# tuanir/fantoch

Hardware: AMD Instinct MI355X
Metric: region configs evaluated/sec (1/2/4/8 GPUs), synthetic 64-region planet n=7 f=1,2 (higher is better)
Workload: dtype u32

## Files before the change

fantoch_amd/csrc/bote_capi.hip:

```cpp
#include <hip/hip_runtime.h>

#include <algorithm>
#include <cmath>
#include <cstring>
#include <mutex>
#include <string>
#include <map>
#include <memory>
#include <vector>

#include "../../include/bote_hip.h"
#include "bote_host.hpp"
#include "bote_kernels.hpp"

using bote::EvalArgs;
using bote::Rec;
using bote::SingleArgs;

using namespace bote::host;

namespace {

thread_local std::string g_err;

// ... 85 lines not shown
  const bote_planet* p = nullptr;
  uint32_t n = 0, ns = 0, nc = 0, n_obj = 0, K = 0;
  EvalArgs args{};
  uint32_t grid = 0, bd = 0;
  size_t shm = 0;
  DBuf srv, cli, binom, top, tmp0, tmp1, result, counters;
  DBuf top_alt, counters_alt;
  hipEvent_t ev0 = nullptr, ev1 = nullptr;
  hipEvent_t last0 = nullptr, last1 = nullptr;
  hipEvent_t done = nullptr;
  std::vector<std::pair<hipEvent_t, hipEvent_t>> evpool;
  size_t ev_used = 0;
  bool launched = false;
  bool fast = false;
  bool group = false;
  bool def_obj = false;
  bote::FastArgs fargs{};
  uint32_t fgrid = 0;
  size_t fshm = 0;
  uint32_t xgrid = 0;
  DBuf cqt, rqt, queue, qcount, lowtab;
  DBuf dbg;
  DBuf pstats;
  struct Chunks {
    std::vector<uint64_t> host;
    std::vector<uint64_t> state;
    DBuf dev, sdev;
    uint32_t n = 0;
  };
  std::map<std::pair<uint64_t, uint64_t>, std::unique_ptr<Chunks>> chunks;
  std::map<std::pair<uint64_t, uint64_t>, std::unique_ptr<Chunks>> samples;
  DBuf smin, tseed;
  DBuf kbound;
  mutable std::vector<std::shared_ptr<const GroupWalk>> walks;
  DBuf wctr;
  uint64_t last_rb = 0, last_re = 0;
  hipStream_t last_stream = nullptr;
  uint64_t result_bytes() const { return (uint64_t)n_obj * bote::KP * 16 + 16; }
};

namespace {
constexpr uint64_t QUEUE_CAP = 1ull << 20;

#ifndef BOTE_CHUNKS_PER_WAVE
#define BOTE_CHUNKS_PER_WAVE 32
#endif
}

struct DevGuard {
  int dev = -1;
  DevGuard() {
    if (hipGetDevice(&dev) != hipSuccess) dev = -1;
  }
  ~DevGuard() {
    if (dev >= 0) (void)hipSetDevice(dev);
  }
  DevGuard(const DevGuard&) = delete;
  DevGuard& operator=(const DevGuard&) = delete;
};

extern "C" {

const char* bote_last_error(void) { return g_err.c_str(); }

int bote_device_count(int* out) {
  if (!out) return fail(BOTE_E_ARG, "out is null");
// ... 894 lines not shown
  s->last0 = e0 ? *e0 : s->ev0;
  s->last1 = e1 ? *e1 : s->ev1;
  HIP_TRY(hipEventRecord(s->last0, st));
  HIP_TRY(bote::launch_eval(a, s->n, false, s->grid, s->bd, s->shm, st));
  HIP_TRY(hipEventRecord(s->last1, st));
  return merge_chain(s, s->grid, st);
}

static int sample_seed(bote_sweep* s, bote::FastArgs& f, uint64_t rb, uint64_t re, hipStream_t st) {
  const uint32_t nwaves = s->fgrid * (s->fargs.gbd / 64);
  const uint32_t nsamp = sample_count(rb, re, binom_u64(s->ns, s->n), nwaves, s->K);
  if (!nsamp) return BOTE_OK;
  auto key = std::make_pair(rb, re);
  auto it = s->samples.find(key);
  if (it == s->samples.end()) {
    if (s->samples.size() >= 16) {
      if (s->last_stream) HIP_TRY(hipStreamSynchronize(s->last_stream));
      HIP_TRY(hipStreamSynchronize(st));
      s->samples.clear();
    }
    if (s->n - 3 > 16) return BOTE_OK;
    auto c = std::make_unique<bote_sweep::Chunks>();
    c->n = nsamp;
    c->host = sample_starts(rb, re, nsamp);
    if (!chunk_states(c->host.data(), nsamp, s->n, s->ns, c->state)) return fail(BOTE_E_ARG, "sample rank out of range");
    if (c->dev.alloc(c->host.size() * 8) != hipSuccess || c->sdev.alloc(c->state.size() * 8) != hipSuccess)
      return fail(BOTE_E_NOMEM, "hipMalloc sample chunks");
    HIP_TRY(hipMemcpyAsync(c->dev.p, c->host.data(), c->host.size() * 8, hipMemcpyHostToDevice, st));
    HIP_TRY(hipMemcpyAsync(c->sdev.p, c->state.data(), c->state.size() * 8, hipMemcpyHostToDevice, st));
    it = s->samples.emplace(key, std::move(c)).first;
  }
  const bote_sweep::Chunks* c = it->second.get();
  const uint32_t slots = nwaves >= s->K ? nwaves : nsamp;
  if (s->smin.reserve((size_t)s->n_obj * slots * 8) != hipSuccess || s->tseed.reserve(bote::MAXOBJ * 8) != hipSuccess)
    return fail(BOTE_E_NOMEM, "hipMalloc top-K seed");
  if (slots != nwaves || slots == nsamp) HIP_TRY(hipMemsetAsync(s->smin.p, 0xFF, (size_t)s->n_obj * slots * 8, st));
  bote::FastArgs fs = f;
  fs.smin = s->smin.as<uint64_t>();
  fs.tseed = nullptr;
  fs.wchunks = c->dev.as<uint64_t>();
  fs.wstate = c->sdev.as<uint64_t>();
  fs.nwchunks = nsamp;
  fs.ssteps = 1;
  fs.smin_wave = slots == nwaves && slots != nsamp ? 1u : 0u;
  fs.wctr = f.wctr + 256;
  HIP_TRY(bote::launch_group(fs, s->n, s->def_obj, s->fgrid, s->fshm, st));
  HIP_TRY(bote::launch_seed(fs.smin, fs.smin_wave ? nwaves : nsamp, s->n_obj, s->K, s->tseed.as<uint64_t>(), st));
  f.tseed = s->tseed.as<uint64_t>();
  return BOTE_OK;
}

static int launch_fast_path(bote_sweep* s, uint64_t rb, uint64_t re, hipStream_t st) {
  bote::FastArgs f = s->fargs;
  f.rb = rb;
  f.re = re;
  f.runlen = sweep_runlen(re - rb, s->fgrid, bote::FAST_BD);
  if (s->group) {
    const bote_sweep::Chunks* ch = nullptr;
    int crc = sweep_chunks(s, rb, re, st, &ch);
    if (crc) return crc;
    f.nwchunks = ch ? ch->n : 0;
    f.wchunks = ch ? ch->dev.as<uint64_t>() : nullptr;
    f.wstate = ch && !ch->state.empty() ? ch->sdev.as<uint64_t>() : nullptr;
    if (f.nwchunks) {
      if (!s->wctr.p && s->wctr.alloc(16 * 128) != hipSuccess) return fail(BOTE_E_NOMEM, "hipMalloc work counters");
      f.wctr = s->wctr.as<unsigned int>();
      f.wshards = s->fgrid % 8 == 0 ? 8u : 1u;
    }
  }
  f.kbound = nullptr;
  if (s->group && s->n_obj && s->K && wide_merge(s->fgrid + s->xgrid, s->grid)) {
    if (!s->kbound.p && s->kbound.alloc(bote::MAXOBJ * 8) != hipSuccess) return fail(BOTE_E_NOMEM, "hipMalloc K-th key bound");
    f.kbound = s->kbound.as<unsigned long long>();
  }
  HIP_TRY(bote::launch_zero_ctl(s->counters.as<unsigned long long>(), s->qcount.as<unsigned long long>(),
                                f.nwchunks ? f.wctr : nullptr, s->counters_alt.as<unsigned long long>(), f.kbound, st));
  if (s->group && f.nwchunks && s->n_obj && s->K) {
    int src = sample_seed(s, f, rb, re, st);
    if (src) return src;
  }
  hipEvent_t *e0 = nullptr, *e1 = nullptr;
  int rc;
  if ((rc = timing_slot(s, e0, e1))) return rc;
  s->last0 = *e0;
  s->last1 = *e1;
  if (s->group) HIP_TRY(bote::launch_group(f, s->n, s->def_obj, s->fgrid, s->fshm, st, *e0, *e1));
  else HIP_TRY(bote::launch_fast(f, s->n, s->fgrid, s->fshm, st, *e0, *e1));
  EvalArgs a = s->args;
  a.rank_list = s->queue.as<uint64_t>();
  a.rank_count = s->qcount.as<unsigned long long>();
  a.rb = 0;
  a.re = QUEUE_CAP;
  a.runlen = 1;
  a.out_top = s->n_obj ? s->top.as<Rec>() + (size_t)s->fgrid * s->n_obj * bote::KP : nullptr;
  HIP_TRY(bote::launch_eval(a, s->n, false, s->xgrid, s->bd, s->shm, st));
  EvalArgs g = s->args;
  g.rb = rb;
  g.re = re;
  g.runlen = sweep_runlen(re - rb, s->grid, s->bd);
  g.out_top = s->n_obj ? s->top_alt.as<Rec>() : nullptr;
  g.out_counters = s->counters_alt.as<unsigned long long>();
  g.run_if_over = s->qcount.as<unsigned long long>();
  g.over_cap = QUEUE_CAP;
  HIP_TRY(bote::launch_eval(g, s->n, false, s->grid, s->bd, s->shm, st));
  return merge_chain(s, s->fgrid + s->xgrid, st, s->qcount.as<unsigned long long>(), s->grid, f.kbound);
}

int bote_sweep_launch(bote_sweep* s, uint64_t rank_begin, uint64_t rank_end, void* hip_stream) {
  DevGuard dev_guard;
// ... 382 lines not shown
```

fantoch_amd/csrc/bote_group.hip:

```cpp
#include "bote_fast.hpp"
#include "bote_launch.hpp"

#define AS3 __attribute__((address_space(3)))

namespace bote {

constexpr int GROUP_MAX_BD = 1024;
#ifndef BOTE_GROUP_WAVES
#define BOTE_GROUP_WAVES 5
#endif
#ifndef BOTE_GROUP_WAVES_PERM
#define BOTE_GROUP_WAVES_PERM 4
#endif

__host__ __device__ constexpr int cmax(int a, int b) { return a > b ? a : b; }
template <bool B>
struct BoolC {
  static constexpr bool value = B;
};

template <int N>
struct GCfg {
  using QC = QCfg<N>;
  static constexpr int F = N - 3;
// ... 174 lines not shown
  return (float)__longlong_as_double((long long)tkey) * (1.0f + 0x1p-10f);
}

template <int KA, int KY, class T>
__device__ __forceinline__ void merge_top4(const T* A, const T* y, T* L) {
  static_assert(KA >= 1 && KY >= 1 && KA + KY >= 4 && KA <= 4 && KY <= 4, "4 smallest of KA + KY >= 4 entries");
  T B[4];
#pragma unroll
  for (int i = 0; i < 4; ++i) {
    const int j = 3 - i;
    if (i < KA && j < KY) B[i] = __builtin_elementwise_min(A[i < KA ? i : 0], y[j < KY ? j : 0]);
    else if (i < KA) B[i] = A[i < KA ? i : 0];
    else B[i] = y[j < KY ? j : 0];
  }
  auto ce = [&](int a, int b) {
    const T lo = __builtin_elementwise_min(B[a], B[b]);
    B[b] = __builtin_elementwise_max(B[a], B[b]);
    B[a] = lo;
  };
  ce(0, 2);
  ce(1, 3);
  ce(0, 1);
  ce(2, 3);
#pragma unroll
  for (int i = 0; i < 4; ++i) L[i] = B[i];
}

template <int KA, int KY, int KO, class T>
__device__ __forceinline__ void merge_k(const T* A, const T* y, T* L) {
  if constexpr (KO == 4 && KA + KY >= 4) merge_top4<KA, KY>(A, y, L);
  else merge_lists<KA, KY, KO>(A, y, L);
}

__device__ __forceinline__ void wave_topk(const TopkLds& t, int* lock, uint32_t nc, int n_obj, uint32_t K,
                                          const uint64_t (&key)[MAXOBJ], const bool (&ok)[MAXOBJ], uint64_t rank) {
  const uint32_t lane = threadIdx.x & 63;
  const int KL = (int)K;
  if (lane == 0) {
    while (atomicCAS(lock, 0, 1) != 0) __builtin_amdgcn_s_sleep(2);
  }
  __builtin_amdgcn_wave_barrier();
  __builtin_amdgcn_fence(__ATOMIC_ACQUIRE, "workgroup");
  const uint32_t rlo = (uint32_t)rank, rhi = (uint32_t)(rank >> 32);
#pragma unroll
  for (int o = 0; o < MAXOBJ; ++o) {
    if (o >= n_obj) break;
    Rec* top = t.top + o * KL;
    const Rec mine = Rec{key[o], rank};
    const bool p = ok[o] && rec_lt(mine, t.thr[o]);
    const uint64_t m = __ballot(p);
    if (m == 0) continue;
    const bool h0 = (int)lane < KL, h1 = (int)lane + 64 < KL;
    const Rec x0 = h0 ? top[lane] : rec_max(), x1 = h1 ? top[lane + 64] : rec_max();
    int r0 = (int)lane, r1 = (int)lane + 64;
    int rc = p ? lower_bound_rec(top, KL, mine) : 0;
    const uint32_t klo = (uint32_t)key[o], khi = (uint32_t)(key[o] >> 32);
    for (uint64_t mm = m; mm; mm &= mm - 1) {
      const int src = __builtin_ctzll(mm);
      const uint64_t ck = ((uint64_t)(uint32_t)__builtin_amdgcn_readlane(khi, src) << 32) |
                          (uint32_t)__builtin_amdgcn_readlane(klo, src);
      const uint64_t cr = ((uint64_t)(uint32_t)__builtin_amdgcn_readlane(rhi, src) << 32) |
                          (uint32_t)__builtin_amdgcn_readlane(rlo, src);
      const Rec c = Rec{ck, cr};
      r0 += rec_lt(c, x0);
      r1 += rec_lt(c, x1);
      rc += rec_lt(c, mine);
    }
    if (h0 && r0 < KL) t.tmp[r0] = x0;
    if (h1 && r1 < KL) t.tmp[r1] = x1;
    if (p && rc < KL) t.tmp[rc] = mine;
    wave_sync();
#pragma unroll
    for (int h = 0; h < KP / 64; ++h)
      if ((int)lane + 64 * h < KL) top[lane + 64 * h] = t.tmp[lane + 64 * h];
    wave_sync();
    if (lane == 0 && rec_lt(top[K - 1], t.thr[o])) {
      t.thr[o] = top[K - 1];
      if (o == 0) lock[1] = score_tlo(top[K - 1].key, nc);
      if (o == 3) lock[2] = __float_as_int(cov_tf32(top[K - 1].key));
    }
    wave_sync();
  }
  __builtin_amdgcn_fence(__ATOMIC_RELEASE, "workgroup");
  if (lane == 0) atomicExch(lock, 0);
}

template <class FX, class FY>
__device__ __forceinline__ int cov2_sign(float Vx, uint32_t Sx, float Vy, uint32_t Sy, const FX& dVx, const FY& dVy) {
  const float fx = (float)Sx, fy = (float)Sy;
  const float x = Vx * (fy * fy), y = Vy * (fx * fx);
  const float d = x - y, tol = 0x1p-18f * fmaxf(x, y);
  if (d < -tol) return -1;
  if (d > tol) return 1;
  const double sx = (double)Sx, sy = (double)Sy;
  const double X = dVx() * (sy * sy), Y = dVy() * (sx * sx);
  const double D = X - Y, T = 0x1p-32 * fmax(X, Y);
  return D < -T ? -1 : (D > T ? 1 : 0);
}

template <class FX, class FY>
__device__ __forceinline__ int cov2_sign_ge(float Vx, uint32_t Sx, float Vy, uint32_t Sy, const FX& dVx, const FY& dVy) {
  const float fx = (float)Sx, fy = (float)Sy;
  const float x = Vx * (fy * fy), y = Vy * (fx * fx);
  constexpr float c = 1.0f - 0x1p-18f;
  if (x * c >= y) return 1;
  if (x < y * c) return -1;
  const double sx = (double)Sx, sy = (double)Sy;
  const double X = dVx() * (sy * sy), Y = dVy() * (sx * sx);
  const double D = X - Y, T = 0x1p-32 * fmax(X, Y);
  return D < -T ? -1 : (D > T ? 1 : 0);
}

__device__ __forceinline__ float u64_to_f32(uint64_t x) {
  return __builtin_fmaf((float)(uint32_t)(x >> 32), 0x1p32f, (float)(uint32_t)x);
}

constexpr uint32_t GROUP_UNROLL = 4;
#ifndef BOTE_BIN_FIRST
#define BOTE_BIN_FIRST 0
#endif
#ifndef BOTE_BIN_FIRST_XK
#define BOTE_BIN_FIRST_XK 1
#endif
constexpr uint32_t BIN_UB = 4;
template <int N, bool DEF, bool SI, bool RXC, bool XK, bool BN = false>
__global__ void __launch_bounds__(XK ? GROUP_XK_MAX_BD : GROUP_MAX_BD,
                                  XK ? BOTE_GROUP_WAVES_XK : (GCfg<N>::PERM ? BOTE_GROUP_WAVES_PERM : BOTE_GROUP_WAVES))
    sweep_group_kernel(FastArgs a) {
  const bool sid = SI || a.srv_identity;
  constexpr bool S32 = SI;
  const bool use_rx = GCfg<N>::RX && (SI ? RXC : a.grx != 0);
  using QC = QCfg<N>;
  using GC = GCfg<N>;
  constexpr int NL = QC::NL;
  constexpr int NLW = NL <= 2 ? 1 : 2;
  constexpr int F = GC::F;
  constexpr int FP = GC::FP;
  constexpr int KQ = GC::KQ;
  constexpr int PV = Pow2<N - 1>::v;
  constexpr int PF = Pow2<F>::v;
  constexpr bool PERM = GC::PERM;
  constexpr bool BIN = XK || (PERM && BN);
  constexpr bool BIN_FIRST = BIN && (XK ? BOTE_BIN_FIRST_XK : BOTE_BIN_FIRST);
  static_assert(!XK || (PERM && DEF), "the extended key set runs on the PERM kernels with the default objectives");
  using QT = QTab<N, XK>;
  constexpr int NT = QT::NT;
  extern __shared__ __align__(16) unsigned char smem[];
  size_t off[16];
  group_layout(a, N, NLW, KQ, PERM, off);
  const uint32_t LB = lds_base(smem);
  const uint32_t qtab = LB + (uint32_t)off[0];
  const uint32_t cqt = LB + (uint32_t)off[1];
  const uint32_t rqt = LB + (uint32_t)(a.rq_separate ? off[2] : off[1]);
  uint32_t* srv = (uint32_t*)(smem + off[3]);
  uint2* lrec = (uint2*)(smem + off[4]);
  uint64_t* cs2 = (uint64_t*)(smem + off[5]);
  double* vcol = (double*)(smem + off[6]);
  float* vcol32 = (float*)(smem + off[7]);
  const uint64_t* binom = a.binom;
  TopkLds tk;
  tk.top = (Rec*)(smem + off[9]);
  tk.cand = (Rec*)(smem + off[10]);
  tk.tmp = (Rec*)(smem + off[11]);
// ... 50 lines not shown
  __syncthreads();

  const uint32_t nc = a.nc, nq = nc >> 2, rem = nc & 3;
  const uint32_t qlane = qtab + tid * 4;
  const uint32_t lines = qtab + wid * lines_wave_bytes(a);
  const uint32_t keys = lines + a.gslots * cstride;
  const uint32_t gl = LB + (uint32_t)off[8] + wid * gline_bytes(a, N, KQ);
  const uint32_t rxt = gl;
  const uint32_t mfl = gl + gline_rx_bytes(a, N);
  const uint32_t upk = mfl + cstride;
  const uint32_t fS1 = upk + FP * KQ * 4;
  const uint32_t fVf = fS1 + F * 4;
  const double pnc1 = a.p_fmean * (double)nc, pnc2 = a.p_emean * (double)nc;
  uint64_t valid_cnt = 0;
  const uint32_t dofs = uni(LB + (uint32_t)off[15] + wid * 512u - 2u * (LB + (uint32_t)off[14] + wid * (N * 256u)));
  auto digest_add = [&](uint32_t binb_, uint64_t d) {
    uint32_t ad;
    asm("v_lshl_add_u32 %0, %1, 1, %2" : "=v"(ad) : "v"(binb_), "s"(dofs));
    __hip_atomic_fetch_add((AS3 uint64_t*)(uintptr_t)ad, d, __ATOMIC_RELAXED, __HIP_MEMORY_SCOPE_WAVEFRONT);
  };

  bool static_done = false;
  const uint32_t wsh = a.wshards ? a.wshards : 1u, wx = blockIdx.x % wsh;
  unsigned int* const tctr = a.wctr + 32 * wx;
  uint32_t cnext = 0;
  if (a.nwchunks && lane == 0) cnext = atomicAdd(tctr, 1u);
  for (;;) {
  uint64_t r, rend;
  uint32_t chunk = ~0u;
  if (a.nwchunks) {
    const uint32_t c = wx + wsh * uni(cnext);
    if (c >= a.nwchunks) break;
    if (lane == 0) cnext = atomicAdd(tctr, 1u);
    chunk = c;
    PSTAT(a, 13, true);
    r = uni64(a.wchunks[c]);
    rend = a.smin ? min(r + 64ull * a.ssteps, a.re) : uni64(a.wchunks[c + 1]);
    GASSERT(a, a.rb <= r && r <= rend && rend <= a.re, 0);
  } else {
    if (static_done) break;
    static_done = true;
    const uint64_t nwaves = (uint64_t)gridDim.x * WPB;
    const uint64_t gw = (uint64_t)blockIdx.x * WPB + wid;
    const uint64_t total = a.re - a.rb;
    r = uni64(a.rb + (uint64_t)(((unsigned __int128)total * gw) / nwaves));
    rend = uni64(a.rb + (uint64_t)(((unsigned __int128)total * (gw + 1)) / nwaves));
  }

  if (r < rend) {
    uint32_t hq[F];
    uint64_t base = 0;
    if (a.wstate && chunk != ~0u) {
      const uint64_t* st = a.wstate + 4 * (size_t)chunk;
      base = uni64(st[0]);
      const uint64_t b0 = uni64(st[1]), b1 = uni64(st[2]);
#pragma unroll
      for (int k = 0; k < F; ++k) hq[k] = (uint32_t)((k < 8 ? b0 >> (8 * k) : b1 >> (8 * (k - 8))) & 0xFFu);
    } else {
      uint32_t p[N];
      colex_unrank<N>(binom, a.ns, r, p);
#pragma unroll
      for (int k = 0; k < F; ++k) {
        hq[k] = uni(p[3 + k]);
        base += binom[hq[k] * (N + 1) + (k + 4)];
      }
      base = uni64(base);
// ... 1053 lines not shown
        if (a.smin) {
          const int nobj = XK ? 8 : (DEF ? 5 : a.n_obj);
#pragma unroll
          for (int o = 0; o < MAXOBJ; ++o) {
            if (o >= nobj) break;
            uint64_t v = ok[o] ? key[o] : ~0ull;
#pragma unroll
            for (int d = 32; d >= 1; d >>= 1) {
              const uint64_t w = ((uint64_t)(uint32_t)__shfl_xor((int)(v >> 32), d) << 32) |
                                 (uint32_t)__shfl_xor((int)(uint32_t)v, d);
              v = w < v ? w : v;
            }
            uint32_t ch = uni(chunk);
            asm volatile("" : "+s"(ch));
            const size_t slot = a.smin_wave ? (size_t)o * gridDim.x * WPB + (size_t)blockIdx.x * WPB + wid
                                            : (size_t)o * a.nwchunks + ch;
            if (lane == (a.smin_wave ? (uint32_t)o : 0u) && v != ~0ull)
              atomicMin((unsigned long long*)&a.smin[slot], v);
          }
        } else if (!ABLATE(a, 4)) {
          const int nobj = XK ? 8 : (DEF ? 5 : a.n_obj);
          uint64_t th[MAXOBJ];
#pragma unroll
          for (int o = 0; o < MAXOBJ; ++o)
            if (o < nobj) {
              const uint2 t = l64(thra + 16u * o);
              th[o] = ((uint64_t)t.y << 32) | t.x;
            }
          bool pass = false;
#pragma unroll
          for (int o = 0; o < MAXOBJ; ++o)
            if (o < nobj) pass = pass || (ok[o] && key[o] <= th[o]);
          PSTAT(a, 11, pass);
          if (__ballot(pass)) wave_topk(tk, lock, a.nc, nobj, a.K, key, ok, rank);
        }
        r += len;
        left -= len;
      }
      if (r >= rend || a.smin) break;
      {
        int js = F;
#pragma unroll
        for (int k = F - 1; k >= 0; --k) {
          const uint32_t nxt = (k == F - 1) ? a.ns : hq[k + 1];
          if (hq[k] + 1 < nxt) js = k;
        }
        base = 0;
#pragma unroll
        for (int k = 0; k < F; ++k) {
          hq[k] = uni(k < js ? (uint32_t)(3 + k) : (k == js ? hq[k] + 1 : hq[k]));
          base += binom[hq[k] * (N + 1) + (k + 4)];
        }
        base = uni64(base);
        low = 0;
      }
      wave_sync();
    }
  }
  wave_sync();
  }
  if (a.smin) return;
  if (valid_cnt && lane == 0) atomicAdd(&a.out_counters[0], (unsigned long long)valid_cnt);
  const uint64_t digest = *(const AS3 uint64_t*)(uintptr_t)(LB + (uint32_t)off[15] + tid * 8);
  if (digest) atomicAdd(&a.out_counters[1], (unsigned long long)digest);
  __syncthreads();
  Rec* dst = a.out_top + (size_t)blockIdx.x * a.n_obj * KP;
  if (a.kbound) {
    if (tid < a.n_obj) {
      const Rec kth = tk.top[tid * a.K + a.K - 1];
      uint64_t b = ~0ull;
      if (!(kth.key == ~0ull && kth.rank == ~0ull)) {
        b = atomicMin(&a.kbound[tid], (unsigned long long)kth.key);
        b = b < kth.key ? b : kth.key;
      } else {
        b = __hip_atomic_load(&a.kbound[tid], __ATOMIC_RELAXED, __HIP_MEMORY_SCOPE_AGENT);
      }
      tk.thr[tid].key = b;
    }
    __syncthreads();
    for (uint32_t i = tid; i < (uint32_t)a.n_obj * a.K; i += BD) {
      const uint32_t o = i / a.K, e = i % a.K;
      const uint64_t b = tk.thr[o].key;
      const Rec r = tk.top[i];
      const bool in = !(r.key == ~0ull && r.rank == ~0ull) && r.key <= b;
      bool prev = true;
      if (e) {
        const Rec q = tk.top[i - 1];
        prev = !(q.key == ~0ull && q.rank == ~0ull) && q.key <= b;
      }
      if (in) dst[o * KP + e] = r;
      else if (prev) dst[o * KP + e] = rec_max();
    }
    return;
  }
  for (uint32_t i = tid; i < (uint32_t)a.n_obj * KP; i += BD) {
    const uint32_t o = i / KP, e = i % KP;
    dst[i] = e < a.K ? tk.top[o * a.K + e] : rec_max();
  }
}

static bool group_si(const FastArgs& a) { return a.srv_identity && a.want_digest && a.ft_metric == 2 && a.s32 && a.v32; }

bool group_supports_keys(uint32_t n, uint32_t bd) { return n >= 4 && n <= 7 && group_uses_lines(n) && bd <= GROUP_XK_MAX_BD; }

template <int N, bool XK>
static const void* group_fn_n(const FastArgs& a, bool def) {
  if constexpr (XK) {
    return group_si(a) ? (a.grx ? (const void*)sweep_group_kernel<N, true, true, true, true>
                                : (const void*)sweep_group_kernel<N, true, true, false, true>)
// ... 45 lines not shown
```

fantoch_amd/csrc/bote_kernels.hip:

```cpp
#include <atomic>
#include "bote_kernels.hpp"
#include "bote_launch.hpp"

namespace bote {

struct Smem {
  uint32_t* mat;
  uint32_t* clioff;
  uint32_t* srv;
  uint64_t* cs;
  uint64_t* binom;
  uint32_t* qtab;
  TopkLds tk;
};

__host__ __device__ inline size_t align_up(size_t x, size_t a) { return (x + a - 1) / a * a; }

__host__ __device__ inline size_t smem_layout(const EvalArgs& a, int N, int NLW, uint32_t BD, bool topk,
                                              size_t* off) {
  size_t o = 0;
  off[0] = o; o += (size_t)a.R * a.R * 4;
  off[1] = o; o += (size_t)a.nc * 4;
  off[2] = o; o += (size_t)a.ns * 4;
  o = align_up(o, 16);
// ... 1016 lines not shown
  __syncthreads();
  for (uint32_t i = tid; i < (uint32_t)KP; i += WIDE_BD) out[i] = i < have && i < KK ? buf[i] : rec_max();
}
#undef WIDE_T

hipError_t launch_merge_wide(const Rec* src, uint32_t n_lists, const Rec* alt, uint32_t alt_lists, uint64_t list_stride,
                             const unsigned long long* sel, uint64_t cap, const unsigned long long* kbound, Rec* dst,
                             uint32_t n_obj, uint32_t K, const unsigned long long* csrc, const unsigned long long* calt,
                             uint64_t* cdst, hipStream_t st) {
  if (n_lists > (uint32_t)(WIDE_BD * WIDE_LISTS_PER_THREAD) || alt_lists > (uint32_t)(WIDE_BD * WIDE_LISTS_PER_THREAD))
    return hipErrorInvalidValue;
  const size_t shm = merge_wide_smem();
  static std::atomic<uint64_t> done{0};
  int dev = 0;
  hipError_t e = hipGetDevice(&dev);
  if (e != hipSuccess) return e;
  const uint64_t bit = 1ull << (dev & 63);
  if (!(done.load(std::memory_order_relaxed) & bit)) {
    e = hipFuncSetAttribute((const void*)merge_wide_kernel, hipFuncAttributeMaxDynamicSharedMemorySize, (int)shm);
    if (e != hipSuccess) return e;
    done.fetch_or(bit, std::memory_order_relaxed);
  }
  hipLaunchKernelGGL(merge_wide_kernel, dim3(n_obj), dim3(WIDE_BD), shm, st, src, n_lists, list_stride, dst, alt,
                     alt_lists, sel, cap, kbound, K, csrc, calt, cdst);
  return hipGetLastError();
}

__global__ void pick_counters_kernel(const unsigned long long* src, const unsigned long long* alt,
                                     const unsigned long long* sel, uint64_t cap, uint64_t* dst) {
  if (threadIdx.x < 2) dst[threadIdx.x] = (*sel > cap ? alt : src)[threadIdx.x];
}

__global__ void zero_ctl_kernel(unsigned long long* counters, unsigned long long* qcount, unsigned int* wctr,
                                unsigned long long* counters_alt, unsigned long long* kbound) {
  const uint32_t t = threadIdx.x;
  if (t < 2) counters[t] = 0;
  if (t == 2) *qcount = 0;
  if (t >= 4 && t < 6) counters_alt[t - 4] = 0;
  if (t >= 8 && t < 24 && wctr) wctr[32 * (t - 8)] = 0;
  if (t >= 32 && t < 32 + MAXOBJ && kbound) kbound[t - 32] = ~0ull;
}

hipError_t launch_zero_ctl(unsigned long long* counters, unsigned long long* qcount, unsigned int* wctr,
                           unsigned long long* counters_alt, unsigned long long* kbound, hipStream_t st) {
  hipLaunchKernelGGL(zero_ctl_kernel, dim3(1), dim3(64), 0, st, counters, qcount, wctr, counters_alt, kbound);
  return hipGetLastError();
}

__global__ void __launch_bounds__(1024) seed_kernel(const uint64_t* smin, uint32_t nsamp, uint32_t K, uint64_t* tseed) {
  __shared__ uint32_t hist[256];
  __shared__ uint64_t sel[3];
  __shared__ uint64_t red[2][16];
  __shared__ uint64_t few[64];
  __shared__ uint32_t nfew;
  const uint32_t o = blockIdx.x, tid = threadIdx.x, BD = blockDim.x;
  if (nsamp < K || K == 0) {
    if (tid == 0) tseed[o] = ~0ull;
    return;
  }
  const uint64_t* x = smin + (size_t)o * nsamp;
  constexpr int RP = 32;
  const bool inreg = nsamp <= (uint32_t)RP * BD;
  uint64_t xr[RP];
#pragma unroll
  for (int i = 0; i < RP; ++i) {
    const uint32_t k = tid + (uint32_t)i * BD;
    xr[i] = inreg && k < nsamp ? x[k] : ~0ull;
  }
  uint64_t va = ~0ull, vo = 0;
  if (inreg) {
#pragma unroll
    for (int i = 0; i < RP; ++i)
      if (tid + (uint32_t)i * BD < nsamp) {
        va &= xr[i];
        vo |= xr[i];
      }
  } else {
    for (uint32_t k = tid; k < nsamp; k += BD) {
      va &= x[k];
      vo |= x[k];
    }
  }
#pragma unroll
  for (int d = 32; d >= 1; d >>= 1) {
    va &= (uint64_t)__shfl_xor((long long)va, d);
    vo |= (uint64_t)__shfl_xor((long long)vo, d);
  }
  if ((tid & 63) == 0) {
    red[0][tid >> 6] = va;
    red[1][tid >> 6] = vo;
  }
  __syncthreads();
  if (tid == 0) {
    uint64_t a = ~0ull, b = 0;
    for (uint32_t w = 0; w < (BD >> 6); ++w) {
      a &= red[0][w];
      b |= red[1][w];
    }
    const uint64_t diff = a ^ b;
    const int top = diff ? 63 - __clzll(diff) : -1;
    const int pass0 = top < 0 ? -1 : top / 8;
    sel[0] = pass0 < 0 ? a : (pass0 == 7 ? 0 : a >> (8 * (pass0 + 1)));
    sel[1] = K;
    red[0][0] = (uint64_t)(int64_t)pass0;
  }
  __syncthreads();
  const int pass0 = (int)(int64_t)red[0][0];
  for (int pass = pass0; pass >= 0; --pass) {
    if (tid < 256) hist[tid] = 0;
    __syncthreads();
    const uint64_t prefix = sel[0];
    const int sh = 8 * pass;
    auto count = [&](uint64_t v) {
      if (pass == 7 || (v >> (sh + 8)) == prefix) atomicAdd(&hist[(v >> sh) & 0xFFu], 1u);
    };
    if (inreg) {
#pragma unroll
      for (int i = 0; i < RP; ++i)
        if (tid + (uint32_t)i * BD < nsamp) count(xr[i]);
    } else {
      for (uint32_t k = tid; k < nsamp; k += BD) count(x[k]);
    }
    __syncthreads();
    if (tid < 64) {
      uint32_t c[4], s = 0;
#pragma unroll
      for (int b = 0; b < 4; ++b) c[b] = hist[4 * tid + b];
#pragma unroll
      for (int b = 0; b < 4; ++b) s += c[b];
      uint32_t incl = s;
#pragma unroll
      for (int d = 1; d < 64; d <<= 1) {
        const uint32_t y = __shfl_up(incl, d);
        if ((int)tid >= d) incl += y;
      }
      const uint64_t need = sel[1];
      uint32_t before = incl - s;
      int digit = -1;
      uint64_t left = 0;
#pragma unroll
// ... 8 lines not shown
        sel[0] = (sel[0] << 8) | (uint64_t)digit;
        sel[1] = left;
        sel[2] = hist[digit];
      }
      if (tid == 0) nfew = 0;
    }
    __syncthreads();
    if (pass > 0 && sel[2] <= 64) {
      const uint64_t pfx = sel[0];
      const int shb = 8 * pass;
      auto push = [&](uint64_t v) {
        if ((v >> shb) == pfx) few[atomicAdd(&nfew, 1u)] = v;
      };
      if (inreg) {
#pragma unroll
        for (int i = 0; i < RP; ++i)
          if (tid + (uint32_t)i * BD < nsamp) push(xr[i]);
      } else {
        for (uint32_t k = tid; k < nsamp; k += BD) push(x[k]);
      }
      __syncthreads();
      if (tid < 64) {
        const uint32_t nb = nfew, need = (uint32_t)sel[1];
        const uint64_t v = tid < nb ? few[tid] : ~0ull;
        uint32_t lt = 0, le = 0;
        for (uint32_t j = 0; j < nb; j += 4) {
#pragma unroll
          for (uint32_t u = 0; u < 4; ++u) {
            const uint64_t y = few[j + u];
            lt += (uint32_t)(j + u < nb && y < v);
            le += (uint32_t)(j + u < nb && y <= v);
          }
        }
        if (tid < nb && lt < need && need <= le) tseed[o] = v;
      }
      return;
    }
  }
  if (tid == 0) tseed[o] = sel[0];
}

hipError_t launch_seed(const uint64_t* smin, uint32_t nsamp, uint32_t n_obj, uint32_t K, uint64_t* tseed,
                       hipStream_t st) {
  hipLaunchKernelGGL(seed_kernel, dim3(n_obj), dim3(1024), 0, st, smin, nsamp, K, tseed);
  return hipGetLastError();
}

hipError_t launch_pick_counters(const unsigned long long* src, const unsigned long long* alt,
                                const unsigned long long* sel, uint64_t cap, uint64_t* dst, hipStream_t st) {
  hipLaunchKernelGGL(pick_counters_kernel, dim3(1), dim3(64), 0, st, src, alt, sel, cap, dst);
  return hipGetLastError();
}

__global__ void sum_counters_kernel(const uint64_t* src, uint32_t n, uint64_t stride, uint64_t off, uint64_t* dst) {
  if (threadIdx.x < 2) {
    uint64_t s = 0;
    for (uint32_t i = 0; i < n; ++i) s += src[i * stride + off + threadIdx.x];
    dst[threadIdx.x] = s;
  }
}

hipError_t launch_sum_counters(const uint64_t* src, uint32_t n, uint64_t stride, uint64_t off, uint64_t* dst,
                               hipStream_t st) {
  hipLaunchKernelGGL(sum_counters_kernel, dim3(1), dim3(64), 0, st, src, n, stride, off, dst);
  return hipGetLastError();
}

hipError_t launch_single(const SingleArgs& a, int mode, hipStream_t st) {
  size_t shm = align_up((size_t)a.R * a.R * 4 + a.R, 16) + (size_t)a.R * 4;
  hipError_t e = hipFuncSetAttribute((const void*)single_kernel, hipFuncAttributeMaxDynamicSharedMemorySize, (int)shm);
  if (e != hipSuccess) return e;
  hipLaunchKernelGGL(single_kernel, dim3(1), dim3(256), shm, st, a, mode);
// ... 10 lines not shown
```

fantoch_amd/csrc/bote_kernels.hpp:

```cpp
#pragma once
#include "bote_device.hpp"

namespace bote {

constexpr int NSLOT = 10;
constexpr int G_MERGE_LISTS = 8;
enum { SLOT_AF1 = 0, SLOT_FF1 = 1, SLOT_AF2 = 2, SLOT_FF2 = 3, SLOT_E = 4 };
enum { OBJ_SCORE = 0, OBJ_MEAN = 1, OBJ_COV = 2 };

struct EvalArgs {
  const uint32_t* mat;
  uint32_t R;
  const uint32_t* srv;
  uint32_t ns;
  const uint32_t* cli;
  uint32_t nc;
  int srv_sorted;
  const uint32_t* cfgs;
  const uint64_t* rank_list;
  const unsigned long long* rank_count;
  uint64_t rb, re;
  uint32_t runlen;
  const uint64_t* binom;
  int want_score;
  double p_fmean, p_emean, p_fair;
  int ft_metric;
  uint32_t keys;
  uint32_t* out_vals;
  uint32_t* out_leader;
  uint64_t* out_s1;
  uint64_t* out_s2;
  double* out_mean;
  double* out_cov;
// ... 34 lines not shown
  const uint2* cqt;
  const uint2* rqt;
  int rq_separate;
  uint32_t R, cq_quads, rq_quads;
  uint32_t cq_stride, rq_stride;
  const uint32_t* srv;
  uint32_t ns;
  int srv_identity;
  uint32_t nc;
  const uint64_t* binom;
  uint64_t rb, re;
  uint32_t runlen;
  uint32_t s2_flush;
  uint32_t g_flush;
  uint32_t k_flush;
  uint32_t gbd;
  uint32_t gqsh;
  uint32_t gslots;
  uint32_t grx;
  uint32_t keys;
  uint32_t gbins;
  uint32_t s32;
  uint32_t v32;
  const uint64_t* wchunks;
  uint32_t nwchunks;
  unsigned int* wctr;
  uint32_t wshards;
  const uint64_t* wstate;
  uint64_t* smin;
  const uint64_t* tseed;
  uint32_t ssteps;
  uint32_t smin_wave;
  unsigned long long* kbound;
  int want_score, p_int;
  int64_t p1i, p2i;
  int32_t m1_lo, m1_hi, m2_lo, m2_hi;
  double p_fmean, p_emean;
  int ft_metric;
  int n_obj;
  uint32_t obj_kind[MAXOBJ];
  uint32_t obj_slot[MAXOBJ];
  uint32_t K;
  Rec* out_top;
  unsigned long long* out_counters;
  int want_digest;
  const uint32_t* lowtab;
  uint64_t* queue;
  unsigned long long* queue_count;
  uint64_t queue_cap;
#ifdef BOTE_DEBUG
  unsigned int* dbg_flag;
  uint64_t lowtab_n;
#endif
#ifdef BOTE_PATHSTATS
  unsigned long long* pstats;
#endif
#ifdef BOTE_ABLATION
  uint32_t ablate;
#endif
};
#ifdef BOTE_DEBUG
#define GASSERT(a, cond, code)                                                    \
  do {                                                                            \
    if (!(cond)) atomicOr((a).dbg_flag, 1u << (code));                            \
  } while (0)
#else
// ... 17 lines not shown
#else
#define ABLATE(a, bit) false
#endif
size_t fast_smem_bytes(const FastArgs& a, uint32_t n);
int fast_occupancy(uint32_t n, size_t shm);
hipError_t launch_fast(const FastArgs& a, uint32_t n, uint32_t grid, size_t shm, hipStream_t st, hipEvent_t e0 = nullptr,
                       hipEvent_t e1 = nullptr);
size_t group_smem_bytes(const FastArgs& a, uint32_t n);
bool group_uses_lines(uint32_t n);
#ifndef BOTE_GROUP_WAVES_XK
#define BOTE_GROUP_WAVES_XK 4
#endif
constexpr uint32_t GROUP_XK_MAX_BD = 256 * BOTE_GROUP_WAVES_XK;
bool group_supports_keys(uint32_t n, uint32_t bd);
int group_occupancy(const FastArgs& a, uint32_t n, size_t shm, bool def_objectives);
hipError_t launch_group(const FastArgs& a, uint32_t n, bool def_objectives, uint32_t grid, size_t shm, hipStream_t st,
                        hipEvent_t e0 = nullptr, hipEvent_t e1 = nullptr);

size_t eval_smem_bytes(const EvalArgs& a, uint32_t n, uint32_t bd, bool topk);
int eval_occupancy(uint32_t n, bool full, uint32_t bd, size_t shm, bool keys = false);
hipError_t launch_eval(const EvalArgs& a, uint32_t n, bool full, uint32_t grid, uint32_t bd, size_t shm,
                       hipStream_t st);
hipError_t launch_merge(const Rec* src, uint32_t n_lists, uint64_t list_stride, Rec* dst, uint64_t out_stride,
                        uint32_t n_obj, hipStream_t st);
constexpr uint32_t WIDE_MERGE_LISTS = 4096;
hipError_t launch_merge_wide(const Rec* src, uint32_t n_lists, const Rec* alt, uint32_t alt_lists, uint64_t list_stride,
                             const unsigned long long* sel, uint64_t cap, const unsigned long long* kbound, Rec* dst,
                             uint32_t n_obj, uint32_t K, const unsigned long long* csrc, const unsigned long long* calt,
                             uint64_t* cdst, hipStream_t st);
hipError_t launch_merge_sel(const Rec* src, uint32_t n_lists, const Rec* alt, uint32_t alt_lists, uint64_t list_stride,
                            const unsigned long long* sel, uint64_t cap, Rec* dst, uint64_t out_stride, uint32_t n_obj,
                            hipStream_t st);
hipError_t launch_zero_ctl(unsigned long long* counters, unsigned long long* qcount, unsigned int* wctr,
                           unsigned long long* counters_alt, unsigned long long* kbound, hipStream_t st);
hipError_t launch_seed(const uint64_t* smin, uint32_t nsamp, uint32_t n_obj, uint32_t K, uint64_t* tseed,
                       hipStream_t st);
hipError_t launch_pick_counters(const unsigned long long* src, const unsigned long long* alt,
                                const unsigned long long* sel, uint64_t cap, uint64_t* dst, hipStream_t st);

hipError_t launch_sum_counters(const uint64_t* src, uint32_t n, uint64_t stride, uint64_t off, uint64_t* dst,
                               hipStream_t st);
struct LqArgs {
  const uint32_t* mat;
  uint32_t R;
  const uint32_t* srv;
  uint32_t ns;
  const uint32_t* cli;
  uint32_t nc;
  const uint32_t* cfgs;
  const uint64_t* binom;
  uint64_t rank_begin, ncfg;
  const uint32_t* qs;
  uint32_t nq;
  uint32_t* out_vals;
  uint64_t* out_sum;
  uint64_t* out_sumsq;
};
size_t lq_smem_bytes(const LqArgs& a, uint32_t n);
hipError_t launch_leaderless_q(const LqArgs& a, uint32_t n, uint32_t grid, size_t shm, hipStream_t st);

struct ChainHostLevel {
  uint32_t cnt, n;
  const uint64_t* mask;
  const double* score;
  const double* mean;
};
hipError_t chain_search(const ChainHostLevel* lv, uint32_t ns, int ft_metric, double min_dec, uint64_t max_out,
// ... 7 lines not shown
```

Measured before the change: 48.83 billion.

## Share a device-wide key histogram to tighten per-workgroup top-K thresholds

```diff
diff --git a/fantoch_amd/csrc/bote_bound.hpp b/fantoch_amd/csrc/bote_bound.hpp
--- /dev/null
+++ b/fantoch_amd/csrc/bote_bound.hpp
@@ -0,0 +1,56 @@
+#pragma once
+#include <cstdint>
+
+#if defined(__HIPCC__) || defined(__CUDACC__)
+#define BOTE_HD __host__ __device__ inline
+#else
+#define BOTE_HD inline
+#endif
+
+namespace bote {
+
+constexpr uint32_t BOUND_NB = 256;
+constexpr uint32_t BOUND_OFF = 64;
+
+struct BoundPlan {
+  uint64_t base;
+  uint64_t top;
+  uint32_t shift;
+};
+
+BOTE_HD BoundPlan bound_plan(uint64_t base, uint64_t top) {
+  BoundPlan p{base, top, BOUND_OFF};
+  if (top == ~0ull || base > top) return p;
+  const uint64_t d = top - base;
+  uint32_t s = 0;
+  while (s < 63 && (d >> s) > BOUND_NB - 1) ++s;
+  p.shift = s;
+  return p;
+}
+
+BOTE_HD bool bound_on(const BoundPlan& p) { return p.shift < BOUND_OFF; }
+
+BOTE_HD uint32_t bound_bin(const BoundPlan& p, uint64_t k) {
+  if (!bound_on(p) || k <= p.base) return 0;
+  const uint64_t j = (k - p.base) >> p.shift;
+  return j < BOUND_NB - 1 ? (uint32_t)j : BOUND_NB - 1;
+}
+
+BOTE_HD uint64_t bound_edge(const BoundPlan& p, uint32_t j) {
+  if (!bound_on(p)) return ~0ull;
+  const uint64_t jt = (p.top - p.base) >> p.shift;
+  if (j >= jt) return p.top;
+  return p.base + (((uint64_t)j + 1) << p.shift) - 1;
+}
+
+BOTE_HD uint64_t bound_from_hist(const BoundPlan& p, const uint32_t* hist, uint32_t K) {
+  if (!bound_on(p) || K == 0) return ~0ull;
+  uint64_t sum = 0;
+  for (uint32_t j = 0; j < BOUND_NB; ++j) {
+    sum += hist[j];
+    if (sum >= K) return bound_edge(p, j);
+  }
+  return ~0ull;
+}
+
+}
diff --git a/fantoch_amd/csrc/bote_capi.hip b/fantoch_amd/csrc/bote_capi.hip
--- a/fantoch_amd/csrc/bote_capi.hip
+++ b/fantoch_amd/csrc/bote_capi.hip
@@ -141,6 +141,7 @@
   std::map<std::pair<uint64_t, uint64_t>, std::unique_ptr<Chunks>> samples;
   DBuf smin, tseed;
   DBuf kbound;
+  DBuf bhist;
   mutable std::vector<std::shared_ptr<const GroupWalk>> walks;
   DBuf wctr;
   uint64_t last_rb = 0, last_re = 0;
@@ -1101,7 +1102,7 @@
   }
   const bote_sweep::Chunks* c = it->second.get();
   const uint32_t slots = nwaves >= s->K ? nwaves : nsamp;
-  if (s->smin.reserve((size_t)s->n_obj * slots * 8) != hipSuccess || s->tseed.reserve(bote::MAXOBJ * 8) != hipSuccess)
+  if (s->smin.reserve((size_t)s->n_obj * slots * 8) != hipSuccess || s->tseed.reserve(3 * bote::MAXOBJ * 8) != hipSuccess)
     return fail(BOTE_E_NOMEM, "hipMalloc top-K seed");
   if (slots != nwaves || slots == nsamp) HIP_TRY(hipMemsetAsync(s->smin.p, 0xFF, (size_t)s->n_obj * slots * 8, st));
   bote::FastArgs fs = f;
@@ -1142,8 +1143,15 @@
     if (!s->kbound.p && s->kbound.alloc(bote::MAXOBJ * 8) != hipSuccess) return fail(BOTE_E_NOMEM, "hipMalloc K-th key bound");
     f.kbound = s->kbound.as<unsigned long long>();
   }
+  f.bhist = nullptr;
+  if (s->group && f.nwchunks && s->n_obj && s->K) {
+    if (!s->bhist.p && s->bhist.alloc(bote::MAXOBJ * bote::BOUND_NB * 4) != hipSuccess)
+      return fail(BOTE_E_NOMEM, "hipMalloc key bound histograms");
+    f.bhist = s->bhist.as<unsigned int>();
+  }
   HIP_TRY(bote::launch_zero_ctl(s->counters.as<unsigned long long>(), s->qcount.as<unsigned long long>(),
-                                f.nwchunks ? f.wctr : nullptr, s->counters_alt.as<unsigned long long>(), f.kbound, st));
+                                f.nwchunks ? f.wctr : nullptr, s->counters_alt.as<unsigned long long>(), f.kbound, f.bhist,
+                                st));
   if (s->group && f.nwchunks && s->n_obj && s->K) {
     int src = sample_seed(s, f, rb, re, st);
     if (src) return src;
diff --git a/fantoch_amd/csrc/bote_group.hip b/fantoch_amd/csrc/bote_group.hip
--- a/fantoch_amd/csrc/bote_group.hip
+++ b/fantoch_amd/csrc/bote_group.hip
@@ -230,10 +230,93 @@
   else merge_lists<KA, KY, KO>(A, y, L);
 }
 
+__device__ __forceinline__ BoundPlan load_plan(const uint64_t* plan, int o) {
+  return BoundPlan{plan[MAXOBJ + o], plan[o], (uint32_t)plan[2 * MAXOBJ + o]};
+}
+
+__device__ __forceinline__ void lower_thr(const TopkLds& t, int* lock, int o, const Rec r, uint32_t nc) {
+  if (!rec_lt(r, t.thr[o])) return;
+  t.thr[o] = r;
+  if (o == 0) lock[1] = score_tlo(r.key, nc);
+  if (o == 3) lock[2] = __float_as_int(cov_tf32(r.key));
+}
+
+static_assert(BOUND_NB == 256, "wave_bound reads 4 bins per lane");
+__device__ __forceinline__ void wave_bound(const unsigned int* bhist, const uint64_t* plan, int n_obj, uint32_t K,
+                                           uint64_t (&edge)[MAXOBJ]) {
+  const uint32_t lane = threadIdx.x & 63;
+  asm volatile("" : "+s"(bhist), "+s"(plan));
+  uint32_t c[MAXOBJ][4];
+#pragma unroll
+  for (int o = 0; o < MAXOBJ; ++o) {
+    if (o >= n_obj) break;
+#pragma unroll
+    for (int b = 0; b < 4; ++b)
+      c[o][b] = __hip_atomic_load(&bhist[o * BOUND_NB + 4 * lane + b], __ATOMIC_RELAXED, __HIP_MEMORY_SCOPE_AGENT);
+  }
+#pragma unroll
+  for (int o = 0; o < MAXOBJ; ++o) {
+    edge[o] = ~0ull;
+    if (o >= n_obj) continue;
+    const BoundPlan pl = load_plan(plan, o);
+    if (!bound_on(pl)) continue;
+    uint32_t s = 0;
+#pragma unroll
+    for (int b = 0; b < 4; ++b) s = min(K, s + min(K, c[o][b]));
+    uint32_t incl = s;
+#pragma unroll
+    for (int d = 1; d < 64; d <<= 1) {
+      const uint32_t y = __shfl_up(incl, d);
+      if ((int)lane >= d) incl = min(K, incl + y);
+    }
+    const uint64_t reach = __ballot(incl >= K);
+    if (reach == 0) continue;
+    const int src = __builtin_ctzll(reach);
+    uint32_t before = __shfl_up(incl, 1);
+    if (lane == 0) before = 0;
+    int j = 3;
+#pragma unroll
+    for (int b = 3; b >= 0; --b) {
+      uint32_t upto = before;
+#pragma unroll
+      for (int bb = 0; bb <= b; ++bb) upto = min(K, upto + min(K, c[o][bb]));
+      if (upto >= K) j = b;
+    }
+    const uint32_t bin = 4u * (uint32_t)src + (uint32_t)__builtin_amdgcn_readlane(j, src);
+    edge[o] = bound_edge(pl, bin);
+  }
+}
+
+__device__ __forceinline__ void wave_refresh(const TopkLds& t, int* lock, uint32_t nc, int n_obj, uint32_t K,
+                                             const unsigned int* bhist, const uint64_t* plan) {
+  const uint32_t lane = threadIdx.x & 63;
+  uint64_t edge[MAXOBJ];
+  wave_bound(bhist, plan, n_obj, K, edge);
+  bool any = false;
+#pragma unroll
+  for (int o = 0; o < MAXOBJ; ++o)
+    if (o < n_obj) any = any || edge[o] < *(volatile uint64_t*)&t.thr[o].key;
+  if (!any) return;
+  if (lane == 0) {
+    while (atomicCAS(lock, 0, 1) != 0) __builtin_amdgcn_s_sleep(2);
+  }
+  __builtin_amdgcn_wave_barrier();
+  __builtin_amdgcn_fence(__ATOMIC_ACQUIRE, "workgroup");
+  if (lane == 0) {
+#pragma unroll
+    for (int o = 0; o < MAXOBJ; ++o)
+      if (o < n_obj && edge[o] != ~0ull) lower_thr(t, lock, o, Rec{edge[o], ~0ull}, nc);
+  }
+  __builtin_amdgcn_fence(__ATOMIC_RELEASE, "workgroup");
+  if (lane == 0) atomicExch(lock, 0);
+}
+
 __device__ __forceinline__ void wave_topk(const TopkLds& t, int* lock, uint32_t nc, int n_obj, uint32_t K,
-                                          const uint64_t (&key)[MAXOBJ], const bool (&ok)[MAXOBJ], uint64_t rank) {
+                                          const uint64_t (&key)[MAXOBJ], const bool (&ok)[MAXOBJ], uint64_t rank,
+                                          unsigned int* bhist, const uint64_t* plan) {
   const uint32_t lane = threadIdx.x & 63;
   const int KL = (int)K;
+  uint32_t pm = 0;
   if (lane == 0) {
     while (atomicCAS(lock, 0, 1) != 0) __builtin_amdgcn_s_sleep(2);
   }
@@ -248,6 +331,7 @@
     const bool p = ok[o] && rec_lt(mine, t.thr[o]);
     const uint64_t m = __ballot(p);
     if (m == 0) continue;
+    pm |= (uint32_t)p << o;
     const bool h0 = (int)lane < KL, h1 = (int)lane + 64 < KL;
     const Rec x0 = h0 ? top[lane] : rec_max(), x1 = h1 ? top[lane + 64] : rec_max();
     int r0 = (int)lane, r1 = (int)lane + 64;
@@ -272,15 +356,21 @@
     for (int h = 0; h < KP / 64; ++h)
       if ((int)lane + 64 * h < KL) top[lane + 64 * h] = t.tmp[lane + 64 * h];
     wave_sync();
-    if (lane == 0 && rec_lt(top[K - 1], t.thr[o])) {
-      t.thr[o] = top[K - 1];
-      if (o == 0) lock[1] = score_tlo(top[K - 1].key, nc);
-      if (o == 3) lock[2] = __float_as_int(cov_tf32(top[K - 1].key));
-    }
+    if (lane == 0) lower_thr(t, lock, o, top[K - 1], nc);
     wave_sync();
   }
   __builtin_amdgcn_fence(__ATOMIC_RELEASE, "workgroup");
   if (lane == 0) atomicExch(lock, 0);
+  if (bhist) {
+    asm volatile("" : "+s"(bhist), "+s"(plan));
+#pragma unroll
+    for (int o = 0; o < MAXOBJ; ++o) {
+      if (o >= n_obj) break;
+      const BoundPlan pl = load_plan(plan, o);
+      if (bound_on(pl) && ((pm >> o) & 1u))
+        __hip_atomic_fetch_add(&bhist[o * BOUND_NB + bound_bin(pl, key[o])], 1u, __ATOMIC_RELAXED, __HIP_MEMORY_SCOPE_AGENT);
+    }
+  }
 }
 
 template <class FX, class FY>
@@ -327,6 +417,7 @@
     sweep_group_kernel(FastArgs a) {
   const bool sid = SI || a.srv_identity;
   constexpr bool S32 = SI;
+  constexpr bool BOUND = !XK;
   const bool use_rx = GCfg<N>::RX && (SI ? RXC : a.grx != 0);
   using QC = QCfg<N>;
   using GC = GCfg<N>;
@@ -443,6 +534,9 @@
     const uint32_t c = wx + wsh * uni(cnext);
     if (c >= a.nwchunks) break;
     if (lane == 0) cnext = atomicAdd(tctr, 1u);
+    if constexpr (BOUND)
+      if (wid == 0 && a.bhist && a.tseed && !a.smin)
+        wave_refresh(tk, lock, a.nc, DEF ? 5 : a.n_obj, a.K, a.bhist, a.tseed);
     chunk = c;
     PSTAT(a, 13, true);
     r = uni64(a.wchunks[c]);
@@ -1562,7 +1656,15 @@
           for (int o = 0; o < MAXOBJ; ++o)
             if (o < nobj) pass = pass || (ok[o] && key[o] <= th[o]);
           PSTAT(a, 11, pass);
-          if (__ballot(pass)) wave_topk(tk, lock, a.nc, nobj, a.K, key, ok, rank);
+#ifdef BOTE_PATHSTATS
+#pragma unroll
+          for (int o = 0; o < MAXOBJ; ++o)
+            if (o < nobj) {
+              PSTAT(a, 16 + o, ok[o] && key[o] <= th[o]);
+              PSTAT(a, 24 + o, ok[o] && rec_lt(Rec{key[o], rank}, tk.thr[o]));
+            }
+#endif
+          if (__ballot(pass)) wave_topk(tk, lock, a.nc, nobj, a.K, key, ok, rank, BOUND && a.tseed ? a.bhist : nullptr, a.tseed);
         }
         r += len;
         left -= len;
@@ -1595,6 +1697,14 @@
   if (digest) atomicAdd(&a.out_counters[1], (unsigned long long)digest);
   __syncthreads();
   Rec* dst = a.out_top + (size_t)blockIdx.x * a.n_obj * KP;
+  if (BOUND && wid == 0 && a.bhist && a.tseed) {
+    uint64_t edge[MAXOBJ];
+    wave_bound(a.bhist, a.tseed, a.n_obj, a.K, edge);
+#pragma unroll
+    for (int o = 0; o < MAXOBJ; ++o)
+      if (o < a.n_obj && lane == 0 && edge[o] < tk.thr[o].key) tk.thr[o] = Rec{edge[o], ~0ull};
+  }
+  __syncthreads();
   if (a.kbound) {
     if (tid < a.n_obj) {
       const Rec kth = tk.top[tid * a.K + a.K - 1];
@@ -1605,6 +1715,7 @@
       } else {
         b = __hip_atomic_load(&a.kbound[tid], __ATOMIC_RELAXED, __HIP_MEMORY_SCOPE_AGENT);
       }
+      b = b < tk.thr[tid].key ? b : tk.thr[tid].key;
       tk.thr[tid].key = b;
     }
     __syncthreads();
diff --git a/fantoch_amd/csrc/bote_kernels.hip b/fantoch_amd/csrc/bote_kernels.hip
--- a/fantoch_amd/csrc/bote_kernels.hip
+++ b/fantoch_amd/csrc/bote_kernels.hip
@@ -1072,30 +1072,38 @@
 }
 
 __global__ void zero_ctl_kernel(unsigned long long* counters, unsigned long long* qcount, unsigned int* wctr,
-                                unsigned long long* counters_alt, unsigned long long* kbound) {
+                                unsigned long long* counters_alt, unsigned long long* kbound, unsigned int* bhist) {
   const uint32_t t = threadIdx.x;
   if (t < 2) counters[t] = 0;
   if (t == 2) *qcount = 0;
   if (t >= 4 && t < 6) counters_alt[t - 4] = 0;
   if (t >= 8 && t < 24 && wctr) wctr[32 * (t - 8)] = 0;
   if (t >= 32 && t < 32 + MAXOBJ && kbound) kbound[t - 32] = ~0ull;
+  if (bhist)
+    for (uint32_t i = t; i < MAXOBJ * BOUND_NB / 4; i += blockDim.x) ((uint4*)bhist)[i] = make_uint4(0, 0, 0, 0);
 }
 
 hipError_t launch_zero_ctl(unsigned long long* counters, unsigned long long* qcount, unsigned int* wctr,
-                           unsigned long long* counters_alt, unsigned long long* kbound, hipStream_t st) {
-  hipLaunchKernelGGL(zero_ctl_kernel, dim3(1), dim3(64), 0, st, counters, qcount, wctr, counters_alt, kbound);
+                           unsigned long long* counters_alt, unsigned long long* kbound, unsigned int* bhist,
+                           hipStream_t st) {
+  hipLaunchKernelGGL(zero_ctl_kernel, dim3(1), dim3(256), 0, st, counters, qcount, wctr, counters_alt, kbound, bhist);
   return hipGetLastError();
 }
 
 __global__ void __launch_bounds__(1024) seed_kernel(const uint64_t* smin, uint32_t nsamp, uint32_t K, uint64_t* tseed) {
   __shared__ uint32_t hist[256];
   __shared__ uint64_t sel[3];
-  __shared__ uint64_t red[2][16];
+  __shared__ uint64_t red[3][16];
   __shared__ uint64_t few[64];
   __shared__ uint32_t nfew;
   const uint32_t o = blockIdx.x, tid = threadIdx.x, BD = blockDim.x;
+  auto publish = [&](uint64_t base, uint64_t top) {
+    tseed[o] = top;
+    tseed[MAXOBJ + o] = base;
+    tseed[2 * MAXOBJ + o] = bound_plan(base, top).shift;
+  };
   if (nsamp < K || K == 0) {
-    if (tid == 0) tseed[o] = ~0ull;
+    if (tid == 0) publish(~0ull, ~0ull);
     return;
   }
   const uint64_t* x = smin + (size_t)o * nsamp;
@@ -1107,36 +1115,43 @@
     const uint32_t k = tid + (uint32_t)i * BD;
     xr[i] = inreg && k < nsamp ? x[k] : ~0ull;
   }
-  uint64_t va = ~0ull, vo = 0;
+  uint64_t va = ~0ull, vo = 0, vm = ~0ull;
   if (inreg) {
 #pragma unroll
     for (int i = 0; i < RP; ++i)
       if (tid + (uint32_t)i * BD < nsamp) {
         va &= xr[i];
         vo |= xr[i];
+        vm = xr[i] < vm ? xr[i] : vm;
       }
   } else {
     for (uint32_t k = tid; k < nsamp; k += BD) {
       va &= x[k];
       vo |= x[k];
+      vm = x[k] < vm ? x[k] : vm;
     }
   }
 #pragma unroll
   for (int d = 32; d >= 1; d >>= 1) {
     va &= (uint64_t)__shfl_xor((long long)va, d);
     vo |= (uint64_t)__shfl_xor((long long)vo, d);
+    const uint64_t wm = (uint64_t)__shfl_xor((long long)vm, d);
+    vm = wm < vm ? wm : vm;
   }
   if ((tid & 63) == 0) {
     red[0][tid >> 6] = va;
     red[1][tid >> 6] = vo;
+    red[2][tid >> 6] = vm;
   }
   __syncthreads();
   if (tid == 0) {
-    uint64_t a = ~0ull, b = 0;
+    uint64_t a = ~0ull, b = 0, m = ~0ull;
     for (uint32_t w = 0; w < (BD >> 6); ++w) {
       a &= red[0][w];
       b |= red[1][w];
-    }
+      m = red[2][w] < m ? red[2][w] : m;
+    }
+    red[2][0] = m;
     const uint64_t diff = a ^ b;
     const int top = diff ? 63 - __clzll(diff) : -1;
     const int pass0 = top < 0 ? -1 : top / 8;
@@ -1146,6 +1161,7 @@
   }
   __syncthreads();
   const int pass0 = (int)(int64_t)red[0][0];
+  const uint64_t least = red[2][0];
   for (int pass = pass0; pass >= 0; --pass) {
     if (tid < 256) hist[tid] = 0;
     __syncthreads();
@@ -1220,12 +1236,12 @@
             le += (uint32_t)(j + u < nb && y <= v);
           }
         }
-        if (tid < nb && lt < need && need <= le) tseed[o] = v;
+        if (tid < nb && lt < need && need <= le) publish(least, v);
       }
       return;
     }
   }
-  if (tid == 0) tseed[o] = sel[0];
+  if (tid == 0) publish(least, sel[0]);
 }
 
 hipError_t launch_seed(const uint64_t* smin, uint32_t nsamp, uint32_t n_obj, uint32_t K, uint64_t* tseed,
diff --git a/fantoch_amd/csrc/bote_kernels.hpp b/fantoch_amd/csrc/bote_kernels.hpp
--- a/fantoch_amd/csrc/bote_kernels.hpp
+++ b/fantoch_amd/csrc/bote_kernels.hpp
@@ -1,4 +1,5 @@
 #pragma once
+#include "bote_bound.hpp"
 #include "bote_device.hpp"
 
 namespace bote {
@@ -99,6 +100,7 @@
   uint32_t ssteps;
   uint32_t smin_wave;
   unsigned long long* kbound;
+  unsigned int* bhist;
   int want_score, p_int;
   int64_t p1i, p2i;
   int32_t m1_lo, m1_hi, m2_lo, m2_hi;
@@ -182,7 +184,8 @@
                             const unsigned long long* sel, uint64_t cap, Rec* dst, uint64_t out_stride, uint32_t n_obj,
                             hipStream_t st);
 hipError_t launch_zero_ctl(unsigned long long* counters, unsigned long long* qcount, unsigned int* wctr,
-                           unsigned long long* counters_alt, unsigned long long* kbound, hipStream_t st);
+                           unsigned long long* counters_alt, unsigned long long* kbound, unsigned int* bhist,
+                           hipStream_t st);
 hipError_t launch_seed(const uint64_t* smin, uint32_t nsamp, uint32_t n_obj, uint32_t K, uint64_t* tseed,
                        hipStream_t st);
 hipError_t launch_pick_counters(const unsigned long long* src, const unsigned long long* alt,
```

Result: no change. 49.04 billion (median of 6 runs) (+0.4%).
